# AdrianoEttari/DiffusionRemoteSensing

Measured on AMD Instinct MI355X. Metric: unet_denoise_steps_per_s, higher is better.
Workload: dtype f16 main + block-scaled fp6 (e2m3) cross terms of tap pairs on the wide 3x3 layers (FL, 11 of 11 launches of the dominant kernel); split bf16 x3 (hi + lo) everywhere else; f32 accumulate

## Files before the change

### diffusionremotesensing_amd/csrc/conv_s2_sp.hip

```cpp
#include <stdio.h>
#include <stdlib.h>

#include "conv_epilogue.h"
#include "mfma_policy.h"

namespace {

__device__ __forceinline__ void copy_weights(char* smem, const TapConv& d, int nck, int GC, int n0, unsigned w_gimage, int tid) {
  const int slots = nck * 36 * GC;
  const char* wsrc = reinterpret_cast<const char*>(d.w);
  for (int i0 = tid; i0 < 2 * slots; i0 += 512 * 8) {
    u32x4 v[8];
#pragma unroll
    for (int u = 0; u < 8; ++u) {
      const int i = i0 + u * 512;
      if (i < 2 * slots) {
        const int im = i >= slots, idx = im ? i - slots : i;
        const int r = idx / GC, j = idx - r * GC;
        v[u] = *reinterpret_cast<const u32x4*>(wsrc + (size_t)im * w_gimage + ((size_t)r * d.Cout + n0 + j) * 16);
      }
    }
#pragma unroll
    for (int u = 0; u < 8; ++u) {
      const int i = i0 + u * 512;
      if (i < 2 * slots) *reinterpret_cast<u32x4*>(smem + (size_t)i * 16) = v[u];
    }
  }
}

template <int NT>
__global__ __launch_bounds__(512, 1) void conv_s2_sp_kernel(TapConv d, int nck, unsigned w_gimage) {
  extern __shared__ __attribute__((aligned(16))) char smem[];
  using P = PolicyBF16X3;
  constexpr int GC = 16 * NT;
  const int tid = threadIdx.x, lane = tid & 63, wave = __builtin_amdgcn_readfirstlane(tid >> 6);
  const int lr = lane & 15, kg = lane >> 4;
  const int ngroups = d.Cout / GC;
  const int xcd = blockIdx.x & 7, j8 = blockIdx.x >> 3, nb8 = gridDim.x >> 3;
  const int grp = j8 % ngroups, member = j8 / ngroups, members = nb8 / ngroups;
  const int n0 = grp * GC;
  const int img = nck * 36 * GC * 16;
  copy_weights(smem, d, nck, GC, n0, w_gimage, tid);
  __syncthreads();

  const int bw = (d.OW + 15) / 16;
  const int rows = d.N * d.OH;
  const int r_lo = (int)((long long)rows * xcd / 8), r_hi = (int)((long long)rows * (xcd + 1) / 8);
  const int Q = (r_hi - r_lo) * bw;
  const int stride = members * 8, first = member * 8 + wave;
  const int my_items = first < Q ? (Q - first + stride - 1) / stride : 0;
  const int S = my_items * nck;
  if (S == 0) return;
  const int half = drs_sp_group_bytes(d.in_cs);
  const char* zero = reinterpret_cast<const char*>(d.zero_line) + kg * 16;
  const char* wbase = smem + ((size_t)kg * GC + lr) * 16;

  struct Taps { typename P::Frag c[3], r[3], e[3]; };
  Taps fa, fb;
  auto issue = [&](int s, Taps& f) __attribute__((always_inline)) {
    const int it = s / nck, c = s - it * nck;
    const int q = first + it * stride;
    const int row = r_lo + q / bw, xb = q - (q / bw) * bw;
    const int n = row / d.OH, y = row - n * d.OH;
    const int px = min(xb * 16 + lr, d.OW - 1);
    const int iy0 = 2 * y - 1, ix0 = 2 * px - 1;
    const char* base = reinterpret_cast<const char*>(d.in) +
                       ((((long long)n * d.H + iy0) * d.W + ix0) * d.in_cs + d.in_co) * 4 + c * 128 + kg * 16;
    const int rowb = d.W * d.in_cs * 4, pixb = d.in_cs * 4;
#pragma unroll
    for (int ky = 0; ky < 3; ++ky) {
      const bool row_ok = ky > 0 || iy0 >= 0;
      const char* pc = row_ok ? base + ky * rowb + pixb : zero;
      const char* pr = row_ok ? base + ky * rowb + 2 * pixb : zero;
      f.c[ky] = typename P::Frag{*reinterpret_cast<const bf16x8*>(pc), *reinterpret_cast<const bf16x8*>(row_ok ? pc + half : zero)};
      f.r[ky] = typename P::Frag{*reinterpret_cast<const bf16x8*>(pr), *reinterpret_cast<const bf16x8*>(row_ok ? pr + half : zero)};
      if (lr == 0) {
        const bool ok = row_ok && ix0 >= 0;
        const char* pe = ok ? base + ky * rowb : zero;
        f.e[ky] = typename P::Frag{*reinterpret_cast<const bf16x8*>(pe), *reinterpret_cast<const bf16x8*>(ok ? pe + half : zero)};
      }
    }
  };
  auto shift_in = [&](const bf16x8& edge, const bf16x8& right) __attribute__((always_inline)) {
    const u32x4 e = __builtin_bit_cast(u32x4, edge), r = __builtin_bit_cast(u32x4, right);
    u32x4 o;
#pragma unroll
    for (int j = 0; j < 4; ++j)
      o[j] = (unsigned)__builtin_amdgcn_update_dpp((int)e[j], (int)r[j], 0x111, 0xf, 0xf, false);
    return __builtin_bit_cast(bf16x8, o);
  };
  f32x4 acc[1][NT];
  float bias8[NT / 2][8];
#pragma unroll
  for (int pr = 0; pr < NT / 2; ++pr) {
    const float4 a = d.bias ? *reinterpret_cast<const float4*>(d.bias + n0 + pr * 32 + kg * 8) : make_float4(0.f, 0.f, 0.f, 0.f);
    const float4 b = d.bias ? *reinterpret_cast<const float4*>(d.bias + n0 + pr * 32 + kg * 8 + 4) : make_float4(0.f, 0.f, 0.f, 0.f);
    bias8[pr][0] = a.x; bias8[pr][1] = a.y; bias8[pr][2] = a.z; bias8[pr][3] = a.w;
    bias8[pr][4] = b.x; bias8[pr][5] = b.y; bias8[pr][6] = b.z; bias8[pr][7] = b.w;
  }
  auto store_row = [&](int n, int y, int x0) __attribute__((always_inline)) {
    const bool lo = lr < 8;
    const int pl = lr & 7;
#pragma unroll
    for (int pr = 0; pr < NT / 2; ++pr) {
      float v[8];
#pragma unroll
      for (int j = 0; j < 4; ++j) { v[j] = acc[0][2 * pr][j] + bias8[pr][j]; v[4 + j] = acc[0][2 * pr + 1][j] + bias8[pr][4 + j]; }
      if (d.relu_pre || d.relu_post) {
#pragma unroll
        for (int j = 0; j < 8; ++j) v[j] = drs_maxf(v[j], 0.f);
      }
      u32x4 H, L;
      drs_sp_split8(v, H, L);
      const u32x4 got = drs_dpp_swap8(lo ? L : H);
#pragma unroll
      for (int h = 0; h < 2; ++h) {
        const int tx = x0 + pl + 8 * h;
        if (tx < d.OW) {
          const size_t opix = ((size_t)n * d.OH + y) * d.OW + tx;
          char* gp = reinterpret_cast<char*>(d.out) + (opix * d.out_cs + d.out_co + n0 + pr * 32) * 4 + (lo ? 0 : 64) + kg * 16;
          drs_store16(gp, (h == 0) ? (lo ? H : got) : (lo ? got : L));
        }
      }
    }
  };
  auto compute = [&](int s, const Taps& f) __attribute__((always_inline)) {
    const int it = s / nck, c = s - it * nck;
    if (c == 0) {
#pragma unroll
      for (int t = 0; t < NT; ++t) acc[0][t] = f32x4{0.f, 0.f, 0.f, 0.f};
    }
    const char* wc = wbase + (size_t)c * 36 * GC * 16;
#pragma unroll
    for (int ky = 0; ky < 3; ++ky) {
      const typename P::Frag left{shift_in(f.e[ky].hi, f.r[ky].hi), shift_in(f.e[ky].lo, f.r[ky].lo)};
#pragma unroll
      for (int kx = 0; kx < 3; ++kx) {
        const typename P::Frag& a = kx == 0 ? left : (kx == 1 ? f.c[ky] : f.r[ky]);
#pragma unroll
        for (int t = 0; t < NT; ++t) {
          const typename P::Frag wf = P::load(wc, (size_t)img, (size_t)((ky * 3 + kx) * 4 * GC + t * 16) * 16);
          acc[0][t] = P::mma(wf, a, acc[0][t]);
        }
      }
      __builtin_amdgcn_sched_barrier(0);
    }
    if (c == nck - 1) {
      const int q = first + it * stride;
      const int row = r_lo + q / bw, xb = q - (q / bw) * bw;
      const int n = row / d.OH, y = row - n * d.OH;
      store_row(n, y, xb * 16);
    }
  };
  issue(0, fa);
  for (int s = 0; s < S; s += 2) {
    if (s + 1 < S) issue(s + 1, fb);
    compute(s, fa);
    if (s + 2 < S) issue(s + 2, fa);
    if (s + 1 < S) compute(s + 1, fb);
  }
}


template <int NT>
__global__ __launch_bounds__(512, 1) void convt_sp_kernel(TapConv d, int nck, unsigned w_gimage) {
  extern __shared__ __attribute__((aligned(16))) char smem[];
  using P = PolicyBF16X3;
  constexpr int GC = 16 * NT;
  const int tid = threadIdx.x, lane = tid & 63, wave = __builtin_amdgcn_readfirstlane(tid >> 6);
  const int lr = lane & 15, kg = lane >> 4;
  const int ngroups = d.Cout / GC;
  const int xcd = blockIdx.x & 7, j8 = blockIdx.x >> 3, nb8 = gridDim.x >> 3;
  const int grp = j8 % ngroups, member = j8 / ngroups, members = nb8 / ngroups;
  const int n0 = grp * GC;
  const int img = nck * 36 * GC * 16;
  copy_weights(smem, d, nck, GC, n0, w_gimage, tid);
  __syncthreads();

  const int bw = d.W / 16;
  const int rows = d.N * (d.H >> 1);
  const int r_lo = (int)((long long)rows * xcd / 8), r_hi = (int)((long long)rows * (xcd + 1) / 8);
  const int Q = (r_hi - r_lo) * bw;
  const int stride = members * 8, first = member * 8 + wave;
  const int my_items = first < Q ? (Q - first + stride - 1) / stride : 0;
  const int S = my_items * nck;
  if (S == 0) return;
  const int half = drs_sp_group_bytes(d.in_cs);
  const char* zero = reinterpret_cast<const char*>(d.zero_line) + kg * 16;
  const char* wbase = smem + ((size_t)kg * GC + lr) * 16;

  struct Rows { typename P::Frag a[3], e[3]; };
  Rows fa, fb;
  auto issue = [&](int s, Rows& f) __attribute__((always_inline)) {
    const int it = s / nck, c = s - it * nck;
    const int q = first + it * stride;
    const int row = r_lo + q / bw, xb = q - (q / bw) * bw;
    const int hh = d.H >> 1;
    const int n = row / hh, y = 2 * (row - n * hh);
    const int px = xb * 16 + lr;
    const char* base = reinterpret_cast<const char*>(d.in) +
                       ((((long long)n * d.H + y) * d.W + px) * d.in_cs + d.in_co) * 4 + c * 128 + kg * 16;
    const int rowb = d.W * d.in_cs * 4, pixb = d.in_cs * 4;
#pragma unroll
    for (int dy = 0; dy < 3; ++dy) {
      const bool row_ok = y + dy < d.H;
      const char* p = row_ok ? base + dy * rowb : zero;
      f.a[dy] = typename P::Frag{*reinterpret_cast<const bf16x8*>(p), *reinterpret_cast<const bf16x8*>(row_ok ? p + half : zero)};
      if (lr == 15) {
        const bool ok = row_ok && px + 1 < d.W;
        const char* pe = ok ? base + dy * rowb + pixb : zero;
        f.e[dy] = typename P::Frag{*reinterpret_cast<const bf16x8*>(pe), *reinterpret_cast<const bf16x8*>(ok ? pe + half : zero)};
      }
    }
  };
  auto shift_in = [&](const bf16x8& edge, const bf16x8& own) __attribute__((always_inline)) {
    const u32x4 e = __builtin_bit_cast(u32x4, edge), r = __builtin_bit_cast(u32x4, own);
    u32x4 o;
#pragma unroll
    for (int j = 0; j < 4; ++j)
      o[j] = (unsigned)__builtin_amdgcn_update_dpp((int)e[j], (int)r[j], 0x101, 0xf, 0xf, false);
    return __builtin_bit_cast(bf16x8, o);
  };
  f32x4 acc[2][4][NT];
  float bias8[NT / 2][8];
#pragma unroll
  for (int pr = 0; pr < NT / 2; ++pr) {
    const float4 a = d.bias ? *reinterpret_cast<const float4*>(d.bias + n0 + pr * 32 + kg * 8) : make_float4(0.f, 0.f, 0.f, 0.f);
    const float4 b = d.bias ? *reinterpret_cast<const float4*>(d.bias + n0 + pr * 32 + kg * 8 + 4) : make_float4(0.f, 0.f, 0.f, 0.f);
    bias8[pr][0] = a.x; bias8[pr][1] = a.y; bias8[pr][2] = a.z; bias8[pr][3] = a.w;
    bias8[pr][4] = b.x; bias8[pr][5] = b.y; bias8[pr][6] = b.z; bias8[pr][7] = b.w;
  }
  auto store_item = [&](int r, int n, int y, int x0) __attribute__((always_inline)) {
    const bool lo = lr < 8;
    const int pl = lr & 7;
#pragma unroll
    for (int ph = 0; ph < 4; ++ph)
#pragma unroll
      for (int pr = 0; pr < NT / 2; ++pr) {
        float v[8];
#pragma unroll
        for (int j = 0; j < 4; ++j) { v[j] = acc[r][ph][2 * pr][j] + bias8[pr][j]; v[4 + j] = acc[r][ph][2 * pr + 1][j] + bias8[pr][4 + j]; }
        u32x4 H, L;
        drs_sp_split8(v, H, L);
        const u32x4 got = drs_dpp_swap8(lo ? L : H);
        const size_t orow = ((size_t)n * d.OH + 2 * y + (ph >> 1)) * d.OW;
#pragma unroll
        for (int h = 0; h < 2; ++h) {
          const size_t opix = orow + 2 * (x0 + pl + 8 * h) + (ph & 1);
          char* gp = reinterpret_cast<char*>(d.out) + (opix * d.out_cs + d.out_co + n0 + pr * 32) * 4 + (lo ? 0 : 64) + kg * 16;
          drs_store16(gp, (h == 0) ? (lo ? H : got) : (lo ? got : L));
        }
      }
  };
  auto compute = [&](int s, const Rows& f) __attribute__((always_inline)) {
    const int it = s / nck, c = s - it * nck;
    if (c == 0) {
#pragma unroll
      for (int r = 0; r < 2; ++r)
#pragma unroll
        for (int ph = 0; ph < 4; ++ph)
#pragma unroll
          for (int t = 0; t < NT; ++t) acc[r][ph][t] = f32x4{0.f, 0.f, 0.f, 0.f};
    }
    const char* wc = wbase + (size_t)c * 36 * GC * 16;
    typename P::Frag right[3];
#pragma unroll
    for (int i = 0; i < 3; ++i) right[i] = typename P::Frag{shift_in(f.e[i].hi, f.a[i].hi), shift_in(f.e[i].lo, f.a[i].lo)};
#pragma unroll
    for (int dy = 0; dy < 2; ++dy) {
#pragma unroll
      for (int dx = 0; dx < 2; ++dx) {
#pragma unroll
        for (int ky = 0; ky < 3; ++ky)
#pragma unroll
          for (int kx = 0; kx < 3; ++kx) {
            if ((ky == 0 ? 1 : 0) != dy || (kx == 0 ? 1 : 0) != dx) continue;
            const int ph = (ky == 1 ? 0 : 1) * 2 + (kx == 1 ? 0 : 1);
#pragma unroll
            for (int t = 0; t < NT; ++t) {
              const typename P::Frag wf = P::load(wc, (size_t)img, (size_t)((ky * 3 + kx) * 4 * GC + t * 16) * 16);
#pragma unroll
              for (int r = 0; r < 2; ++r) acc[r][ph][t] = P::mma(wf, dx == 0 ? f.a[r + dy] : right[r + dy], acc[r][ph][t]);
            }
          }
        __builtin_amdgcn_sched_barrier(0);
      }
    }
    if (c == nck - 1) {
      const int q = first + it * stride;
      const int row = r_lo + q / bw, xb = q - (q / bw) * bw;
      const int hh = d.H >> 1;
      const int n = row / hh, y = 2 * (row - n * hh);
      store_item(0, n, y, xb * 16);
      store_item(1, n, y + 1, xb * 16);
    }
  };
  issue(0, fa);
  for (int s = 0; s < S; s += 2) {
    if (s + 1 < S) issue(s + 1, fb);
    compute(s, fa);
    if (s + 2 < S) issue(s + 2, fa);
    if (s + 1 < S) compute(s + 1, fb);
  }
}

template <int NT, bool CONVT = false>
int s2_launch(const TapConv& d, int nck, unsigned w_gimage, hipStream_t s) {
  auto kern = CONVT ? convt_sp_kernel<2> : conv_s2_sp_kernel<NT>;
  const size_t lds = (size_t)2 * nck * 36 * 16 * NT * 16;
  int num_cu = 0;
  {
    const int rc = drs_kernel_prepare(reinterpret_cast<const void*>(kern), 160 * 1024, &num_cu);
    if (rc) return rc;
  }
  const int ngroups = d.Cout / (16 * NT);
  int per_xcd = num_cu / 8;
  per_xcd = per_xcd / ngroups * ngroups;
  if (per_xcd < ngroups) per_xcd = ngroups;
  DRS_LAUNCH(kern, dim3((unsigned)(8 * per_xcd)), dim3(512), lds, s, d, nck, w_gimage);
  DRS_CHECK_HIP(hipGetLastError());
  return DRS_OK;
}

int s2_tiles(const TapConv& d) {
  const int nck = d.Cin / 32;
  const size_t budget = 156 * 1024;
  if (d.Cout % 64 == 0 && d.Cout <= 64 && (size_t)2 * nck * 36 * 64 * 16 <= budget) return 4;
  if ((size_t)2 * nck * 36 * 32 * 16 <= budget) return 2;
  return 0;
}

}

bool drs_conv_s2_sp_supported(const TapConv& d, int impl) {
  static const int env = getenv("DRS_S2K") ? atoi(getenv("DRS_S2K")) : 1;
  if (!env || impl != DRS_IMPL_MFMA_BF16X3) return false;
  if (!d.in || !d.in_sp || !d.out || !d.out_sp || !d.zero_line || d.mode != 0 || d.ntaps != 9 || d.wtaps_total != 9) return false;
  if (d.in_stride != 2 || d.out_scale != 1 || d.out_oy || d.out_ox) return false;
  for (int i = 0; i < 9; ++i)
    if (d.dy[i] != i / 3 - 1 || d.dx[i] != i % 3 - 1 || d.wtap[i] != i) return false;
  if (d.in2 || d.out2 || d.fuse_out || d.dual || d.gate || d.in_add || d.res || d.sigmoid || d.out_nchw) return false;
  if ((d.H & 1) || (d.W & 1) || d.OH != d.H / 2 || d.OW != d.W / 2 || d.TH != d.OH || d.TW != d.OW) return false;
  if (d.Cin % 32 || d.Cout % 32 || (d.in_cs & 31) || (d.in_co & 31) || (d.out_cs & 31) || (d.out_co & 31)) return false;
  if (d.post_add || d.bias2) return false;
  return s2_tiles(d) != 0;
}

int drs_launch_conv_s2_sp(const TapConv& d, hipStream_t s) {
  const int nck = d.Cin / 32;
  const unsigned w_gimage = (unsigned)((size_t)nck * 9 * 4 * d.Cout * 16);
  return s2_tiles(d) == 4 ? s2_launch<4>(d, nck, w_gimage, s) : s2_launch<2>(d, nck, w_gimage, s);
}

bool drs_convt_sp_supported(const TapConv& d, int impl) {
  static const int env = getenv("DRS_S2K") ? atoi(getenv("DRS_S2K")) : 1;
  if (!env || impl != DRS_IMPL_MFMA_BF16X3) return false;
  if (!d.in || !d.in_sp || !d.out || !d.out_sp || !d.zero_line || d.mode != DRS_TAPMODE_CONVT || d.ntaps != 9 || d.wtaps_total != 9) return false;
  if (d.in_stride != 1 || d.out_scale != 2 || d.out_oy || d.out_ox) return false;
  for (int i = 0; i < 9; ++i)
    if (d.wtap[i] != i) return false;
  if (d.in2 || d.out2 || d.fuse_out || d.dual || d.gate || d.in_add || d.res || d.sigmoid || d.out_nchw) return false;
  if (d.post_add || d.bias2 || d.relu_pre || d.relu_post) return false;
  if ((d.W & 15) || (d.H & 1) || d.OH != 2 * d.H || d.OW != 2 * d.W || d.TH != d.H || d.TW != d.W) return false;
  if (d.Cin % 32 || d.Cout % 32 || (d.in_cs & 31) || (d.in_co & 31) || (d.out_cs & 31) || (d.out_co & 31)) return false;
  return (size_t)2 * (d.Cin / 32) * 36 * 32 * 16 <= 156 * 1024;
}

int drs_launch_convt_sp(const TapConv& d, hipStream_t s) {
  const int nck = d.Cin / 32;
  const unsigned w_gimage = (unsigned)((size_t)nck * 9 * 4 * d.Cout * 16);
  return s2_launch<2, true>(d, nck, w_gimage, s);
}
```

Before: 829.7.

## Compute two output rows per work item in stride-2 conv to share input rows

Adds a two-row variant of the stride-2 3x3 conv kernel. Each wave now loads five input rows and produces two output rows, so the shared middle row is reused. Edge pixels for all rows come from one gather and are spread with DPP row shifts. Bias moves to LDS, the loop is restructured into phased loads interleaved with MFMA, and a heuristic chooses two rows only when there are enough items. The cost is more accumulator registers, possible load imbalance from fewer items, and a larger LDS footprint.

```diff
diff --git a/diffusionremotesensing_amd/csrc/conv_s2_sp.hip b/diffusionremotesensing_amd/csrc/conv_s2_sp.hip
--- a/diffusionremotesensing_amd/csrc/conv_s2_sp.hip
+++ b/diffusionremotesensing_amd/csrc/conv_s2_sp.hip
@@ -28,23 +28,18 @@
   }
 }
 
-template <int NT>
-__global__ __launch_bounds__(512, 1) void conv_s2_sp_kernel(TapConv d, int nck, unsigned w_gimage) {
-  extern __shared__ __attribute__((aligned(16))) char smem[];
+template <int NT, int R>
+__device__ __forceinline__ void s2_items(const TapConv& d, int nck, const char* smem, int member, int members, int n0) {
   using P = PolicyBF16X3;
   constexpr int GC = 16 * NT;
   const int tid = threadIdx.x, lane = tid & 63, wave = __builtin_amdgcn_readfirstlane(tid >> 6);
   const int lr = lane & 15, kg = lane >> 4;
-  const int ngroups = d.Cout / GC;
-  const int xcd = blockIdx.x & 7, j8 = blockIdx.x >> 3, nb8 = gridDim.x >> 3;
-  const int grp = j8 % ngroups, member = j8 / ngroups, members = nb8 / ngroups;
-  const int n0 = grp * GC;
+  const int xcd = blockIdx.x & 7;
   const int img = nck * 36 * GC * 16;
-  copy_weights(smem, d, nck, GC, n0, w_gimage, tid);
-  __syncthreads();
 
   const int bw = (d.OW + 15) / 16;
-  const int rows = d.N * d.OH;
+  const int G = (d.OH + R - 1) / R;
+  const int rows = d.N * G;
   const int r_lo = (int)((long long)rows * xcd / 8), r_hi = (int)((long long)rows * (xcd + 1) / 8);
   const int Q = (r_hi - r_lo) * bw;
   const int stride = members * 8, first = member * 8 + wave;
@@ -55,32 +50,6 @@
   const char* zero = reinterpret_cast<const char*>(d.zero_line) + kg * 16;
   const char* wbase = smem + ((size_t)kg * GC + lr) * 16;
 
-  struct Taps { typename P::Frag c[3], r[3], e[3]; };
-  Taps fa, fb;
-  auto issue = [&](int s, Taps& f) __attribute__((always_inline)) {
-    const int it = s / nck, c = s - it * nck;
-    const int q = first + it * stride;
-    const int row = r_lo + q / bw, xb = q - (q / bw) * bw;
-    const int n = row / d.OH, y = row - n * d.OH;
-    const int px = min(xb * 16 + lr, d.OW - 1);
-    const int iy0 = 2 * y - 1, ix0 = 2 * px - 1;
-    const char* base = reinterpret_cast<const char*>(d.in) +
-                       ((((long long)n * d.H + iy0) * d.W + ix0) * d.in_cs + d.in_co) * 4 + c * 128 + kg * 16;
-    const int rowb = d.W * d.in_cs * 4, pixb = d.in_cs * 4;
-#pragma unroll
-    for (int ky = 0; ky < 3; ++ky) {
-      const bool row_ok = ky > 0 || iy0 >= 0;
-      const char* pc = row_ok ? base + ky * rowb + pixb : zero;
-      const char* pr = row_ok ? base + ky * rowb + 2 * pixb : zero;
-      f.c[ky] = typename P::Frag{*reinterpret_cast<const bf16x8*>(pc), *reinterpret_cast<const bf16x8*>(row_ok ? pc + half : zero)};
-      f.r[ky] = typename P::Frag{*reinterpret_cast<const bf16x8*>(pr), *reinterpret_cast<const bf16x8*>(row_ok ? pr + half : zero)};
-      if (lr == 0) {
-        const bool ok = row_ok && ix0 >= 0;
-        const char* pe = ok ? base + ky * rowb : zero;
-        f.e[ky] = typename P::Frag{*reinterpret_cast<const bf16x8*>(pe), *reinterpret_cast<const bf16x8*>(ok ? pe + half : zero)};
-      }
-    }
-  };
   auto shift_in = [&](const bf16x8& edge, const bf16x8& right) __attribute__((always_inline)) {
     const u32x4 e = __builtin_bit_cast(u32x4, edge), r = __builtin_bit_cast(u32x4, right);
     u32x4 o;
@@ -89,23 +58,33 @@
       o[j] = (unsigned)__builtin_amdgcn_update_dpp((int)e[j], (int)r[j], 0x111, 0xf, 0xf, false);
     return __builtin_bit_cast(bf16x8, o);
   };
-  f32x4 acc[1][NT];
-  float bias8[NT / 2][8];
-#pragma unroll
-  for (int pr = 0; pr < NT / 2; ++pr) {
-    const float4 a = d.bias ? *reinterpret_cast<const float4*>(d.bias + n0 + pr * 32 + kg * 8) : make_float4(0.f, 0.f, 0.f, 0.f);
-    const float4 b = d.bias ? *reinterpret_cast<const float4*>(d.bias + n0 + pr * 32 + kg * 8 + 4) : make_float4(0.f, 0.f, 0.f, 0.f);
-    bias8[pr][0] = a.x; bias8[pr][1] = a.y; bias8[pr][2] = a.z; bias8[pr][3] = a.w;
-    bias8[pr][4] = b.x; bias8[pr][5] = b.y; bias8[pr][6] = b.z; bias8[pr][7] = b.w;
-  }
-  auto store_row = [&](int n, int y, int x0) __attribute__((always_inline)) {
+  f32x4 acc[R][NT];
+  float bias8[R == 1 ? NT / 2 : 1][8];
+  if constexpr (R == 1) {
+#pragma unroll
+    for (int pr = 0; pr < NT / 2; ++pr) {
+      const float4 a = d.bias ? *reinterpret_cast<const float4*>(d.bias + n0 + pr * 32 + kg * 8) : make_float4(0.f, 0.f, 0.f, 0.f);
+      const float4 b = d.bias ? *reinterpret_cast<const float4*>(d.bias + n0 + pr * 32 + kg * 8 + 4) : make_float4(0.f, 0.f, 0.f, 0.f);
+      bias8[pr][0] = a.x; bias8[pr][1] = a.y; bias8[pr][2] = a.z; bias8[pr][3] = a.w;
+      bias8[pr][4] = b.x; bias8[pr][5] = b.y; bias8[pr][6] = b.z; bias8[pr][7] = b.w;
+    }
+  }
+  auto store_row = [&](int r, int n, int y, int x0) __attribute__((always_inline)) {
     const bool lo = lr < 8;
     const int pl = lr & 7;
 #pragma unroll
     for (int pr = 0; pr < NT / 2; ++pr) {
       float v[8];
-#pragma unroll
-      for (int j = 0; j < 4; ++j) { v[j] = acc[0][2 * pr][j] + bias8[pr][j]; v[4 + j] = acc[0][2 * pr + 1][j] + bias8[pr][4 + j]; }
+      if constexpr (R == 1) {
+#pragma unroll
+        for (int j = 0; j < 4; ++j) { v[j] = acc[r][2 * pr][j] + bias8[pr][j]; v[4 + j] = acc[r][2 * pr + 1][j] + bias8[pr][4 + j]; }
+      } else {
+        const float4* bl = reinterpret_cast<const float4*>(smem + 2 * (size_t)img) + pr * 8 + kg * 2;
+        const float4 a = bl[0], b = bl[1];
+        const float b8[8] = {a.x, a.y, a.z, a.w, b.x, b.y, b.z, b.w};
+#pragma unroll
+        for (int j = 0; j < 4; ++j) { v[j] = acc[r][2 * pr][j] + b8[j]; v[4 + j] = acc[r][2 * pr + 1][j] + b8[4 + j]; }
+      }
       if (d.relu_pre || d.relu_post) {
 #pragma unroll
         for (int j = 0; j < 8; ++j) v[j] = drs_maxf(v[j], 0.f);
@@ -124,41 +103,196 @@
       }
     }
   };
-  auto compute = [&](int s, const Taps& f) __attribute__((always_inline)) {
-    const int it = s / nck, c = s - it * nck;
-    if (c == 0) {
-#pragma unroll
-      for (int t = 0; t < NT; ++t) acc[0][t] = f32x4{0.f, 0.f, 0.f, 0.f};
-    }
-    const char* wc = wbase + (size_t)c * 36 * GC * 16;
-#pragma unroll
-    for (int ky = 0; ky < 3; ++ky) {
-      const typename P::Frag left{shift_in(f.e[ky].hi, f.r[ky].hi), shift_in(f.e[ky].lo, f.r[ky].lo)};
-#pragma unroll
-      for (int kx = 0; kx < 3; ++kx) {
-        const typename P::Frag& a = kx == 0 ? left : (kx == 1 ? f.c[ky] : f.r[ky]);
-#pragma unroll
-        for (int t = 0; t < NT; ++t) {
-          const typename P::Frag wf = P::load(wc, (size_t)img, (size_t)((ky * 3 + kx) * 4 * GC + t * 16) * 16);
-          acc[0][t] = P::mma(wf, a, acc[0][t]);
-        }
-      }
-      __builtin_amdgcn_sched_barrier(0);
-    }
-    if (c == nck - 1) {
+  if constexpr (R == 1) {
+    struct Taps { typename P::Frag c[3], r[3], e[3]; };
+    Taps fa, fb;
+    auto issue = [&](int s, Taps& f) __attribute__((always_inline)) {
+      const int it = s / nck, c = s - it * nck;
       const int q = first + it * stride;
       const int row = r_lo + q / bw, xb = q - (q / bw) * bw;
       const int n = row / d.OH, y = row - n * d.OH;
-      store_row(n, y, xb * 16);
-    }
-  };
-  issue(0, fa);
-  for (int s = 0; s < S; s += 2) {
-    if (s + 1 < S) issue(s + 1, fb);
-    compute(s, fa);
-    if (s + 2 < S) issue(s + 2, fa);
-    if (s + 1 < S) compute(s + 1, fb);
-  }
+      const int px = min(xb * 16 + lr, d.OW - 1);
+      const int iy0 = 2 * y - 1, ix0 = 2 * px - 1;
+      const char* base = reinterpret_cast<const char*>(d.in) +
+                         ((((long long)n * d.H + iy0) * d.W + ix0) * d.in_cs + d.in_co) * 4 + c * 128 + kg * 16;
+      const int rowb = d.W * d.in_cs * 4, pixb = d.in_cs * 4;
+#pragma unroll
+      for (int ky = 0; ky < 3; ++ky) {
+        const bool row_ok = ky > 0 || iy0 >= 0;
+        const char* pc = row_ok ? base + ky * rowb + pixb : zero;
+        const char* pr = row_ok ? base + ky * rowb + 2 * pixb : zero;
+        f.c[ky] = typename P::Frag{*reinterpret_cast<const bf16x8*>(pc), *reinterpret_cast<const bf16x8*>(row_ok ? pc + half : zero)};
+        f.r[ky] = typename P::Frag{*reinterpret_cast<const bf16x8*>(pr), *reinterpret_cast<const bf16x8*>(row_ok ? pr + half : zero)};
+        if (lr == 0) {
+          const bool ok = row_ok && ix0 >= 0;
+          const char* pe = ok ? base + ky * rowb : zero;
+          f.e[ky] = typename P::Frag{*reinterpret_cast<const bf16x8*>(pe), *reinterpret_cast<const bf16x8*>(ok ? pe + half : zero)};
+        }
+      }
+    };
+    auto compute = [&](int s, const Taps& f) __attribute__((always_inline)) {
+      const int it = s / nck, c = s - it * nck;
+      if (c == 0) {
+#pragma unroll
+        for (int t = 0; t < NT; ++t) acc[0][t] = f32x4{0.f, 0.f, 0.f, 0.f};
+      }
+      const char* wc = wbase + (size_t)c * 36 * GC * 16;
+#pragma unroll
+      for (int ky = 0; ky < 3; ++ky) {
+        const typename P::Frag left{shift_in(f.e[ky].hi, f.r[ky].hi), shift_in(f.e[ky].lo, f.r[ky].lo)};
+#pragma unroll
+        for (int kx = 0; kx < 3; ++kx) {
+          const typename P::Frag& a = kx == 0 ? left : (kx == 1 ? f.c[ky] : f.r[ky]);
+#pragma unroll
+          for (int t = 0; t < NT; ++t) {
+            const typename P::Frag wf = P::load(wc, (size_t)img, (size_t)((ky * 3 + kx) * 4 * GC + t * 16) * 16);
+            acc[0][t] = P::mma(wf, a, acc[0][t]);
+          }
+        }
+        __builtin_amdgcn_sched_barrier(0);
+      }
+      if (c == nck - 1) {
+        const int q = first + it * stride;
+        const int row = r_lo + q / bw, xb = q - (q / bw) * bw;
+        const int n = row / d.OH, y = row - n * d.OH;
+        store_row(0, n, y, xb * 16);
+      }
+    };
+    issue(0, fa);
+    for (int s = 0; s < S; s += 2) {
+      if (s + 1 < S) issue(s + 1, fb);
+      compute(s, fa);
+      if (s + 2 < S) issue(s + 2, fa);
+      if (s + 1 < S) compute(s + 1, fb);
+    }
+  } else {
+    static_assert(R == 2, "row slots and phases are laid out for two output rows");
+    struct Row { typename P::Frag c, r; };
+    struct Step { const char* base; int c, n, y0, xb, nr; };
+    const int rowb = d.W * d.in_cs * 4, pixb = d.in_cs * 4;
+    auto locate = [&](int s) __attribute__((always_inline)) {
+      Step st;
+      const int it = s / nck;
+      st.c = s - it * nck;
+      const int q = first + it * stride;
+      const int g = r_lo + q / bw;
+      st.xb = q - (q / bw) * bw;
+      st.n = g / G;
+      st.y0 = (g - st.n * G) * R;
+      st.nr = min(R, d.OH - st.y0);
+      const int px = min(st.xb * 16 + lr, d.OW - 1);
+      st.base = reinterpret_cast<const char*>(d.in) +
+                ((((long long)st.n * d.H + 2 * st.y0 - 1) * d.W + 2 * px - 1) * d.in_cs + d.in_co) * 4 + st.c * 128 + kg * 16;
+      return st;
+    };
+    auto load_row = [&](const Step& st, int j, bool live, Row& f) __attribute__((always_inline)) {
+      const bool row_ok = live && j <= 2 * st.nr && (j > 0 || st.y0 > 0);
+      const char* p = row_ok ? st.base + j * rowb : zero;
+      const int px1 = row_ok ? pixb : 0, hf = row_ok ? half : 0;
+      f.c = typename P::Frag{*reinterpret_cast<const bf16x8*>(p + px1), *reinterpret_cast<const bf16x8*>(p + px1 + hf)};
+      f.r = typename P::Frag{*reinterpret_cast<const bf16x8*>(p + 2 * px1), *reinterpret_cast<const bf16x8*>(p + 2 * px1 + hf)};
+    };
+    auto load_edges = [&](const Step& st, bool live, typename P::Frag& e) __attribute__((always_inline)) {
+      const bool ok = live && lr <= 2 * st.nr && (lr > 0 || st.y0 > 0) && st.xb > 0;
+      const int dx = min(st.xb * 16 + lr, d.OW - 1) - st.xb * 16;
+      const char* pe = ok ? st.base + lr * rowb - 2 * dx * pixb : zero;
+      e = typename P::Frag{*reinterpret_cast<const bf16x8*>(pe), *reinterpret_cast<const bf16x8*>(ok ? pe + half : zero)};
+    };
+    auto left_tap = [&](int j, const bf16x8& edges, const bf16x8& right) __attribute__((always_inline)) {
+      const u32x4 e = __builtin_bit_cast(u32x4, edges);
+      u32x4 o;
+#pragma unroll
+      for (int k = 0; k < 4; ++k) {
+        const int v = (int)e[k];
+        o[k] = (unsigned)(j == 1 ? __builtin_amdgcn_update_dpp(0, v, 0x101, 0xf, 0xf, true)
+                        : j == 2 ? __builtin_amdgcn_update_dpp(0, v, 0x102, 0xf, 0xf, true)
+                        : j == 3 ? __builtin_amdgcn_update_dpp(0, v, 0x103, 0xf, 0xf, true)
+                        : j == 4 ? __builtin_amdgcn_update_dpp(0, v, 0x104, 0xf, 0xf, true) : v);
+      }
+      return shift_in(__builtin_bit_cast(bf16x8, o), right);
+    };
+    auto phase = [&](const char* wc, int ky, bool both, const Row& fa, const Row& fb, const typename P::Frag& e) __attribute__((always_inline)) {
+      const typename P::Frag la{left_tap(ky, e.hi, fa.r.hi), left_tap(ky, e.lo, fa.r.lo)};
+      const typename P::Frag lb = both ? typename P::Frag{left_tap(ky + 2, e.hi, fb.r.hi), left_tap(ky + 2, e.lo, fb.r.lo)} : la;
+#pragma unroll
+      for (int kx = 0; kx < 3; ++kx) {
+        const typename P::Frag& a0 = kx == 0 ? la : (kx == 1 ? fa.c : fa.r);
+        const typename P::Frag& a1 = kx == 0 ? lb : (kx == 1 ? fb.c : fb.r);
+#pragma unroll
+        for (int tp = 0; tp < NT; tp += 2) {
+          const typename P::Frag w0 = P::load(wc, (size_t)img, (size_t)((ky * 3 + kx) * 4 * GC + tp * 16) * 16);
+          const typename P::Frag w1 = P::load(wc, (size_t)img, (size_t)((ky * 3 + kx) * 4 * GC + (tp + 1) * 16) * 16);
+#pragma unroll
+          for (int part = 0; part < 3; ++part) {
+            const bf16x8 u0 = part == 0 ? w0.lo : w0.hi, u1 = part == 0 ? w1.lo : w1.hi;
+            const bf16x8 v0 = part == 1 ? a0.lo : a0.hi;
+            acc[0][tp] = __builtin_amdgcn_mfma_f32_16x16x32_bf16(u0, v0, acc[0][tp], 0, 0, 0);
+            acc[0][tp + 1] = __builtin_amdgcn_mfma_f32_16x16x32_bf16(u1, v0, acc[0][tp + 1], 0, 0, 0);
+            if (both) {
+              const bf16x8 v1 = part == 1 ? a1.lo : a1.hi;
+              acc[1][tp] = __builtin_amdgcn_mfma_f32_16x16x32_bf16(u0, v1, acc[1][tp], 0, 0, 0);
+              acc[1][tp + 1] = __builtin_amdgcn_mfma_f32_16x16x32_bf16(u1, v1, acc[1][tp + 1], 0, 0, 0);
+            }
+          }
+        }
+      }
+      __builtin_amdgcn_sched_barrier(0);
+    };
+    Row f0, f1, f3, f4, fm[2];
+    typename P::Frag fe[2];
+    auto step = [&](const Step& st, const Step& nx, bool more, Row& mid, Row& mid_next, const typename P::Frag& e,
+                    typename P::Frag& e_next) __attribute__((always_inline)) {
+      if (st.c == 0) {
+#pragma unroll
+        for (int r = 0; r < R; ++r)
+#pragma unroll
+          for (int t = 0; t < NT; ++t) acc[r][t] = f32x4{0.f, 0.f, 0.f, 0.f};
+      }
+      const char* wc = wbase + (size_t)st.c * 36 * GC * 16;
+      const bool both = st.nr == 2;
+      load_row(nx, 2, more, mid_next);
+      load_edges(nx, more, e_next);
+      if (both) phase(wc, 0, true, f0, mid, e); else phase(wc, 0, false, f0, mid, e);
+      load_row(nx, 0, more, f0);
+      if (both) phase(wc, 1, true, f1, f3, e); else phase(wc, 1, false, f1, f3, e);
+      load_row(nx, 1, more, f1);
+      load_row(nx, 3, more, f3);
+      if (both) phase(wc, 2, true, mid, f4, e); else phase(wc, 2, false, mid, f4, e);
+      load_row(nx, 4, more, f4);
+      if (st.c == nck - 1) {
+        store_row(0, st.n, st.y0, st.xb * 16);
+        if (both) store_row(1, st.n, st.y0 + 1, st.xb * 16);
+      }
+    };
+    Step sa = locate(0), sb;
+    load_row(sa, 0, true, f0); load_row(sa, 2, true, fm[0]); load_edges(sa, true, fe[0]);
+    load_row(sa, 1, true, f1); load_row(sa, 3, true, f3); load_row(sa, 4, true, f4);
+    for (int s = 0; s < S; s += 2) {
+      const bool more1 = s + 1 < S;
+      sb = locate(more1 ? s + 1 : s);
+      step(sa, sb, more1, fm[0], fm[1], fe[0], fe[1]);
+      if (!more1) break;
+      const bool more2 = s + 2 < S;
+      sa = locate(more2 ? s + 2 : s + 1);
+      step(sb, sa, more2, fm[1], fm[0], fe[1], fe[0]);
+    }
+  }
+}
+
+template <int NT>
+__global__ __launch_bounds__(512, 1) void conv_s2_sp_kernel(TapConv d, int nck, unsigned w_gimage, int rows) {
+  extern __shared__ __attribute__((aligned(16))) char smem[];
+  constexpr int GC = 16 * NT;
+  const int ngroups = d.Cout / GC;
+  const int j8 = blockIdx.x >> 3, nb8 = gridDim.x >> 3;
+  const int grp = j8 % ngroups, member = j8 / ngroups, members = nb8 / ngroups;
+  const int n0 = grp * GC;
+  copy_weights(smem, d, nck, GC, n0, w_gimage, threadIdx.x);
+  if (threadIdx.x < GC)
+    reinterpret_cast<float*>(smem + (size_t)2 * nck * 36 * GC * 16)[threadIdx.x] = d.bias ? d.bias[n0 + threadIdx.x] : 0.f;
+  __syncthreads();
+  if (rows == 2) s2_items<NT, 2>(d, nck, smem, member, members, n0);
+  else s2_items<NT, 1>(d, nck, smem, member, members, n0);
 }
 
 
@@ -304,20 +438,34 @@
   }
 }
 
+constexpr bool kS2TwoRows[2] = { true,  true};
+int s2_rows_per_item(const TapConv& d, int NT, int members) {
+  const char* env = getenv("DRS_S2_ROWS");
+  if (env && (atoi(env) == 1 || atoi(env) == 2)) return atoi(env);
+  if (!kS2TwoRows[NT == 4]) return 1;
+  const long long pairs = (long long)d.N * ((d.OH + 1) / 2);
+  return (pairs / 8) * ((d.OW + 15) / 16) >= 8LL * members ? 2 : 1;
+}
+
 template <int NT, bool CONVT = false>
 int s2_launch(const TapConv& d, int nck, unsigned w_gimage, hipStream_t s) {
-  auto kern = CONVT ? convt_sp_kernel<2> : conv_s2_sp_kernel<NT>;
-  const size_t lds = (size_t)2 * nck * 36 * 16 * NT * 16;
+  const void* kern = CONVT ? reinterpret_cast<const void*>(convt_sp_kernel<2>) : reinterpret_cast<const void*>(conv_s2_sp_kernel<NT>);
+  const size_t lds = (size_t)2 * nck * 36 * 16 * NT * 16 + (CONVT ? 0 : 16 * NT * 4);
   int num_cu = 0;
   {
-    const int rc = drs_kernel_prepare(reinterpret_cast<const void*>(kern), 160 * 1024, &num_cu);
+    const int rc = drs_kernel_prepare(kern, 160 * 1024, &num_cu);
     if (rc) return rc;
   }
   const int ngroups = d.Cout / (16 * NT);
   int per_xcd = num_cu / 8;
   per_xcd = per_xcd / ngroups * ngroups;
   if (per_xcd < ngroups) per_xcd = ngroups;
-  DRS_LAUNCH(kern, dim3((unsigned)(8 * per_xcd)), dim3(512), lds, s, d, nck, w_gimage);
+  if (CONVT) {
+    DRS_LAUNCH(convt_sp_kernel<2>, dim3((unsigned)(8 * per_xcd)), dim3(512), lds, s, d, nck, w_gimage);
+  } else {
+    const int rows = s2_rows_per_item(d, NT, per_xcd / ngroups);
+    DRS_LAUNCH(conv_s2_sp_kernel<NT>, dim3((unsigned)(8 * per_xcd)), dim3(512), lds, s, d, nck, w_gimage, rows);
+  }
   DRS_CHECK_HIP(hipGetLastError());
   return DRS_OK;
 }
```

Result: no change. 837.0 (median of 6 runs) (+0.9%).
